# XPixelGroup/DiffBIR

Hardware: NVIDIA B200
Metric: MPix/s end-to-end 50-step restore @512px (higher is better)
Workload: dtype f16 operands / f32 accumulate

## Files before the change

diffbir_b200/csrc/common.cuh:

```cuda
#pragma once
#include <cuda.h>
#include <cuda_runtime.h>
#include <cuda_fp16.h>
#include <cuda_bf16.h>
#include <stdint.h>
#include <stdio.h>

#ifdef DBIR_OPERAND_BF16
typedef __nv_bfloat16 op_t;
typedef __nv_bfloat162 op2_t;
#define DBIR_OPERAND_KIND 0
#define DBIR_UMMA_FMT 1u
__device__ __forceinline__ op_t f2op(float x) { return __float2bfloat16_rn(x); }
__device__ __forceinline__ float op2f(op_t x) { return __bfloat162float(x); }
__device__ __forceinline__ uint32_t pack2(float a, float b) {
  __nv_bfloat162 v = __floats2bfloat162_rn(a, b);
  return *reinterpret_cast<uint32_t*>(&v);
}
__device__ __forceinline__ float2 unpack2(uint32_t u) {
  __nv_bfloat162 v = *reinterpret_cast<__nv_bfloat162*>(&u);
  return __bfloat1622float2(v);
}
#else
typedef __half op_t;
// ... 9 lines not shown
__device__ __forceinline__ float2 unpack2(uint32_t u) {
  __half2 v = *reinterpret_cast<__half2*>(&u);
  return __half22float2(v);
}
#endif

void dbir_set_error(const char* fmt, ...);
#define DBIR_CHECK_CUDA(expr)                                                     \
  do {                                                                            \
    cudaError_t _e = (expr);                                                      \
    if (_e != cudaSuccess) {                                                      \
      dbir_set_error("%s:%d: %s -> %s", __FILE__, __LINE__, #expr,                \
                     cudaGetErrorString(_e));                                     \
      return -1;                                                                  \
    }                                                                             \
  } while (0)
#define DBIR_REQUIRE(cond, ...)                                                   \
  do {                                                                            \
    if (!(cond)) {                                                                \
      dbir_set_error(__VA_ARGS__);                                                \
      return -2;                                                                  \
    }                                                                             \
  } while (0)

int dbir_make_tmap(CUtensorMap* out, const void* base, int rank, const uint64_t* dims,
                   const uint64_t* strides_bytes, const uint32_t* box, int elem_bytes,
                   int swizzle128);
extern "C" int dbir_sm_count(void);

#ifdef __CUDACC__
extern "C" int dbir_pdl_enabled(void);
template <typename... KArgs, typename... Args>
inline cudaError_t dbir_launch_cluster(void (*kernel)(KArgs...), dim3 grid, dim3 block, size_t smem,
                                       cudaStream_t st, unsigned cluster_x, Args&&... args) {
  cudaLaunchConfig_t cfg{};
  cfg.gridDim = grid;
  cfg.blockDim = block;
  cfg.dynamicSmemBytes = smem;
  cfg.stream = st;
  cudaLaunchAttribute attr[2];
  int n = 0;
  if (dbir_pdl_enabled()) {
    attr[n].id = cudaLaunchAttributeProgrammaticStreamSerialization;
    attr[n].val.programmaticStreamSerializationAllowed = 1;
    ++n;
  }
  if (cluster_x > 1) {
    attr[n].id = cudaLaunchAttributeClusterDimension;
    attr[n].val.clusterDim.x = cluster_x;
    attr[n].val.clusterDim.y = 1;
    attr[n].val.clusterDim.z = 1;
    ++n;
  }
  cfg.attrs = attr;
  cfg.numAttrs = n;
  return cudaLaunchKernelEx(&cfg, kernel, static_cast<KArgs>(args)...);
}
template <typename... KArgs, typename... Args>
inline cudaError_t dbir_launch(void (*kernel)(KArgs...), dim3 grid, dim3 block, size_t smem,
                               cudaStream_t st, Args&&... args) {
  return dbir_launch_cluster(kernel, grid, block, smem, st, 1u, static_cast<Args&&>(args)...);
}
__device__ __forceinline__ void pdl_wait() { asm volatile("griddepcontrol.wait;" ::: "memory"); }
__device__ __forceinline__ void pdl_trigger() { asm volatile("griddepcontrol.launch_dependents;" ::: "memory"); }

__device__ __forceinline__ uint32_t smem_u32(const void* p) {
  return static_cast<uint32_t>(__cvta_generic_to_shared(p));
}

__device__ __forceinline__ bool elect_one() {
  uint32_t pred;
  asm volatile(
      "{\n.reg .pred p;\nelect.sync _|p, 0xffffffff;\nselp.u32 %0, 1, 0, p;\n}\n" : "=r"(pred));
  return pred != 0;
}

__device__ __forceinline__ void mbar_init(uint64_t* bar, uint32_t count) {
  asm volatile("mbarrier.init.shared::cta.b64 [%0], %1;" ::"r"(smem_u32(bar)), "r"(count)
               : "memory");
}
__device__ __forceinline__ void fence_mbar_init() {
  asm volatile("fence.mbarrier_init.release.cluster;" ::: "memory");
}
__device__ __forceinline__ void mbar_expect_tx(uint64_t* bar, uint32_t bytes) {
  asm volatile("mbarrier.arrive.expect_tx.shared::cta.b64 _, [%0], %1;" ::"r"(smem_u32(bar)),
               "r"(bytes)
               : "memory");
}
__device__ __forceinline__ void mbar_arrive(uint64_t* bar) {
  asm volatile("mbarrier.arrive.shared::cta.b64 _, [%0];" ::"r"(smem_u32(bar)) : "memory");
}
__device__ __forceinline__ bool mbar_try_wait(uint64_t* bar, uint32_t parity) {
  uint32_t ok;
  asm volatile(
// ... 282 lines not shown
```

diffbir_b200/csrc/gemm_tc.cu:

```cuda
#include "common.cuh"
#include "../../include/diffbir_b200.h"
#include <stdlib.h>
#include <array>
#include <map>
#include <mutex>
#include <utility>
#include <vector>

namespace {

constexpr int BM = 128;
constexpr int BK = 64;
constexpr int A_SUB_BYTES = BM * BK * 2;
constexpr int EPI_TILE_BYTES = 32 * 32 * 4;

struct GemmParams {
  int M, N, num_kb;
  int mode;
  int H, W, NI;
  int bw, bh, bni;
  int tiles_x, tiles_y;
  int cblocks;
  int kw, pad;
  int wbw, wbh;
  int out_kind;
  const float* bias;
  const float* rowvec;
  int rows_per_vec;
  int has_residual;
  float alpha;
  int act;
  float act_param;
  int geglu;
  int bias_per_row;
  int group_span;
  int splits, kb_per_split;
  float* ws;
  unsigned int* tickets;
  long long* dbg;
  float* stats;
  int stats_nslots, stats_rows_per_img, stats_slots_x;
  const char* pf_ptr;
  long long pf_bytes;
};

__device__ __forceinline__ float apply_act(float v, int act, float prm) {
  if (act == 1) return gelu_erf_f(v);
  if (act == 2) return v > 0.f ? v : v * prm;
  return silu_f(v);
}

__device__ __forceinline__ void sts_v4(uint32_t addr, uint32_t a, uint32_t b, uint32_t c, uint32_t d) {
  asm volatile("st.shared.v4.b32 [%0], {%1, %2, %3, %4};" ::"r"(addr), "r"(a), "r"(b), "r"(c), "r"(d) : "memory");
}
__device__ __forceinline__ float4 lds_v4(uint32_t addr) {
  float4 v;
  asm volatile("ld.shared.v4.f32 {%0, %1, %2, %3}, [%4];" : "=f"(v.x), "=f"(v.y), "=f"(v.z), "=f"(v.w) : "r"(addr) : "memory");
  return v;
}
__device__ __forceinline__ void tma_store_2d(const CUtensorMap* m, uint32_t src, int c0, int c1) {
  asm volatile("cp.async.bulk.tensor.2d.global.shared::cta.bulk_group [%0, {%2, %3}], [%1];" ::"l"(
                   reinterpret_cast<uint64_t>(m)), "r"(src), "r"(c0), "r"(c1) : "memory");
}
__device__ __forceinline__ void tma_store_4d(const CUtensorMap* m, uint32_t src, int c0, int c1, int c2, int c3) {
  asm volatile("cp.async.bulk.tensor.4d.global.shared::cta.bulk_group [%0, {%2, %3, %4, %5}], [%1];" ::"l"(
                   reinterpret_cast<uint64_t>(m)), "r"(src), "r"(c0), "r"(c1), "r"(c2), "r"(c3) : "memory");
}
__device__ __forceinline__ void bulk_commit() { asm volatile("cp.async.bulk.commit_group;" ::: "memory"); }
template <int N>
__device__ __forceinline__ void bulk_wait_read() {
  asm volatile("cp.async.bulk.wait_group.read %0;" ::"n"(N) : "memory");
}

struct EpiCtx {
  const CUtensorMap* tm_out;
  const CUtensorMap* tm_res;
  uint32_t epi_base;
  uint32_t res_bar;
  int row0;
  int x, y, n;
  long long stats_base;
  int grp_off;
  __device__ __forceinline__ uint32_t out_buf(int b) const { return epi_base + b * EPI_TILE_BYTES; }
  __device__ __forceinline__ uint32_t res_buf(int b) const { return epi_base + (2 + b) * EPI_TILE_BYTES; }
  __device__ __forceinline__ uint32_t bar(int b) const { return res_bar + b * 8; }
};

__device__ __forceinline__ void mbar_wait_s(uint32_t bar, uint32_t parity) {
  uint32_t ok = 0;
  long long t0 = 0;
// ... 123 lines not shown
    }
    if (lane < ncols)
      *reinterpret_cast<float2*>(p.stats + (e.stats_base + gc0 + lane) * 2) = make_float2(sa, sb);
  }
  if (lane == 0) {
    if (p.mode == 0) tma_store_2d(e.tm_out, e.out_buf(b), gc0, e.row0);
    else tma_store_4d(e.tm_out, e.out_buf(b), gc0, e.x, e.y, e.n);
    bulk_commit();
  }
}

template <int BN, int STAGES, int EW, bool PAIR, int KSUB>
__global__ void __launch_bounds__(64 + 32 * EW, EW == 4 ? 2 : 1)
gemm_tc_kernel(const __grid_constant__ CUtensorMap tma_a, const __grid_constant__ CUtensorMap tma_b,
               const __grid_constant__ CUtensorMap tma_out, const __grid_constant__ CUtensorMap tma_res,
               const GemmParams p) {
  constexpr int B_ROWS = PAIR ? BN / 2 : BN;
  constexpr int B_SUB_BYTES = B_ROWS * BK * 2;
  constexpr int A_STAGE_BYTES = KSUB * A_SUB_BYTES;
  constexpr int B_STAGE_BYTES = KSUB * B_SUB_BYTES;
  constexpr uint32_t TMEM_COLS = BN <= 32 ? 32 : BN <= 64 ? 64 : BN <= 128 ? 128 : 256;
  static_assert(STAGES * (A_STAGE_BYTES + B_STAGE_BYTES) >= EW * 4 * EPI_TILE_BYTES, "epilogue staging must fit in the pipeline stages");
  constexpr int CSTEP = 32 * (EW / 4);
  extern __shared__ uint8_t smem_raw[];
  uint8_t* smem = reinterpret_cast<uint8_t*>((reinterpret_cast<uintptr_t>(smem_raw) + 1023) &
                                             ~static_cast<uintptr_t>(1023));
  uint8_t* sA = smem;
  uint8_t* sB = smem + STAGES * A_STAGE_BYTES;
  uint64_t* full = reinterpret_cast<uint64_t*>(sB + STAGES * B_STAGE_BYTES);
  uint64_t* empty = full + STAGES;
  uint64_t* tmem_full = empty + STAGES;
  uint64_t* res_bars = tmem_full + 1;
  uint32_t* tmem_slot = reinterpret_cast<uint32_t*>(res_bars + 2 * EW);
  uint32_t* split_flag = tmem_slot + 1;

  const int warp = threadIdx.x >> 5;
  const int lane = threadIdx.x & 31;
  const uint32_t cta_rank = PAIR ? cluster_ctarank() : 0u;
  const int m_tile = blockIdx.x;
  const int n_tile = blockIdx.y;
  const int tile_lin = blockIdx.y * gridDim.x + blockIdx.x;
  const int kb0 = blockIdx.z * p.kb_per_split;
  const int kb1 = min(p.num_kb, kb0 + p.kb_per_split);
  long long t_start = 0, t_setup = 0, t_acc = 0;
  if (p.dbg) t_start = clock64();

  int n0 = 0, y0 = 0, x0 = 0;
  if (p.mode == 1) {
    int t = m_tile;
    int tx = t % p.tiles_x; t /= p.tiles_x;
    int ty = t % p.tiles_y; t /= p.tiles_y;
    x0 = tx * p.bw; y0 = ty * p.bh; n0 = t * p.bni;
  }

  int grp_off = 0;
  if (p.group_span > 0) grp_off = ((p.mode == 1 ? n0 : m_tile) / p.group_span) * p.N;

  if (warp == 0 && lane == 0) {
    tma_prefetch_desc(&tma_a);
    tma_prefetch_desc(&tma_b);
    tma_prefetch_desc(&tma_out);
    if (p.has_residual) tma_prefetch_desc(&tma_res);
  }
  if (warp == 1 && lane == 0) {
    for (int s = 0; s < STAGES; ++s) { mbar_init(&full[s], 1); mbar_init(&empty[s], 1); }
    mbar_init(tmem_full, 1);
    for (int i = 0; i < 2 * EW; ++i) mbar_init(&res_bars[i], 1);
    fence_mbar_init();
  }
  if (warp == 2) {
    if constexpr (PAIR) tmem_alloc_pair(tmem_slot, TMEM_COLS);
    else tmem_alloc(tmem_slot, TMEM_COLS);
  }
  tc_fence_before();
  if constexpr (PAIR) cluster_sync_all();
  else __syncthreads();
  tc_fence_after();
// ... 145 lines not shown
      const int vsel = any_row ? __shfl_sync(0xffffffffu, vec_idx, __ffs(vm) - 1) : 0;
      const bool uniform = !p.rowvec || !any_row || __all_sync(0xffffffffu, out_row < 0 || vec_idx == vsel);
      if (uniform) {
        have_pre = true;
#pragma unroll
        for (int i = 0; i < MAX_PRE; ++i) {
          const int col = n_tile * BN + c_first + i * CSTEP + lane;
          float x = 0.f;
          if (c_first + i * CSTEP < BN && col < p.N) {
            if (p.bias) x = __ldg(p.bias + grp_off + col);
            if (p.rowvec && any_row) x += __ldg(p.rowvec + static_cast<long long>(vsel) * p.N + col);
          }
          pre[i] = x;
        }
      }
    }
    constexpr int MAX_G = (BN / 2) / CSTEP + 1;
    float pa[MAX_G], pg[MAX_G];
    if (p.geglu) {
#pragma unroll
      for (int i = 0; i < MAX_G; ++i) {
        const int c = c_first + i * CSTEP + lane;
        const bool live = p.bias && c_first + i * CSTEP < BN / 2 && n_tile * (BN / 2) + c < p.N / 2;
        pa[i] = live ? __ldg(p.bias + grp_off + n_tile * BN + c) : 0.f;
        pg[i] = live ? __ldg(p.bias + grp_off + n_tile * BN + BN / 2 + c) : 0.f;
      }
    }
    mbar_wait(tmem_full, 0);
    tc_fence_after();
    if (p.dbg) t_acc = clock64();
    const uint32_t taddr = tmem_base + (static_cast<uint32_t>(q * 32) << 16);
    e.epi_base = smem_u32(sA) + ew * (4 * EPI_TILE_BYTES);

    constexpr int OUT_COLS = BN;
    const bool finalize = p.splits == 1;
    if (!p.geglu) {
      const int col_base = n_tile * BN;
      if (finalize && p.has_residual) {
#pragma unroll
        for (int c = 0; c < 2; ++c) {
          const int cc = c_first + c * CSTEP;
          if (cc < OUT_COLS && col_base + cc < p.N) epi_issue_residual(p, e, lane, c, col_base + cc);
        }
      }
      int ci = 0;
#pragma unroll 1
      for (int c0 = c_first; c0 < BN; c0 += CSTEP) {
        uint32_t acc[32];
        __syncwarp();
        tmem_ld32(taddr + c0, acc);
        tmem_ld_wait();
        const int gc0 = col_base + c0;
        if (p.splits > 1) {
          float* wcol = p.ws + ((static_cast<long long>(tile_lin) * p.splits + blockIdx.z) * BN + c0) * BM + r;
#pragma unroll
          for (int j = 0; j < 32; ++j) __stcg(wcol + j * BM, __uint_as_float(acc[j]));
          continue;
        }
        if (gc0 >= p.N) continue;
        const int ncols = min(32, p.N - gc0);
        const int ngc = gc0 + 2 * CSTEP;
        float v[32];
#pragma unroll
        for (int j = 0; j < 32; ++j) v[j] = __uint_as_float(acc[j]);
        finish_chunk(p, e, v, lane, ci, gc0, ncols, (c0 + 2 * CSTEP < BN && ngc < p.N) ? ngc : -1, out_row, vec_idx, true,
                     have_pre, pre[(c0 - c_first) / CSTEP]);
        ++ci;
      }
      if (p.splits > 1) {
        __threadfence();
        asm volatile("bar.sync 1, %0;" ::"n"(32 * EW) : "memory");
        if (threadIdx.x == 64) {
          const unsigned int t = atomicAdd(&p.tickets[tile_lin], 1u);
          const bool last = (t == static_cast<unsigned int>(p.splits) - 1);
          if (last) p.tickets[tile_lin] = 0;
          *split_flag = last ? 1u : 0u;
        }
        asm volatile("bar.sync 1, %0;" ::"n"(32 * EW) : "memory");
        if (*split_flag) {
          __threadfence();
          if (p.has_residual) {
#pragma unroll
            for (int c = 0; c < 2; ++c) {
              const int cc = c_first + c * CSTEP;
              if (cc < BN && col_base + cc < p.N) epi_issue_residual(p, e, lane, c, col_base + cc);
            }
          }
          int cj = 0;
#pragma unroll 1
          for (int c0 = c_first; c0 < BN; c0 += CSTEP) {
            const int gc0 = col_base + c0;
            if (gc0 >= p.N) continue;
            const int ncols = min(32, p.N - gc0);
            const int ngc = gc0 + 2 * CSTEP;
            float v[32];
#pragma unroll
            for (int j = 0; j < 32; ++j) v[j] = 0.f;
            for (int z = 0; z < p.splits; ++z) {
              const float* wcol = p.ws + ((static_cast<long long>(tile_lin) * p.splits + z) * BN + c0) * BM + r;
#pragma unroll
              for (int j = 0; j < 32; ++j) v[j] += __ldcg(wcol + j * BM);
            }
            finish_chunk(p, e, v, lane, cj, gc0, ncols, (c0 + 2 * CSTEP < BN && ngc < p.N) ? ngc : -1, out_row, vec_idx, true,
                         have_pre, pre[(c0 - c_first) / CSTEP]);
            ++cj;
          }
        }
      }
    } else {
      constexpr int HB = BN / 2;
      const int n_half = p.N / 2;
      if constexpr (HB % 32 == 0) {
        const uint32_t bb = e.res_buf(0);
#pragma unroll
        for (int i = 0; i < MAX_G; ++i) {
          asm volatile("st.shared.f32 [%0], %1;" ::"r"(bb + (i * 64 + lane) * 4), "f"(pa[i]) : "memory");
          asm volatile("st.shared.f32 [%0], %1;" ::"r"(bb + (i * 64 + 32 + lane) * 4), "f"(pg[i]) : "memory");
        }
        __syncwarp();
        int ci = 0;
#pragma unroll
        for (int i = 0; i < MAX_G; ++i) {
          const int c0 = c_first + i * CSTEP;
          if (c0 >= HB) break;
          uint32_t av[32], ag[32];
          __syncwarp();
          tmem_ld32(taddr + c0, av);
          tmem_ld32(taddr + HB + c0, ag);
          tmem_ld_wait();
          const int gc0 = n_tile * HB + c0;
          if (gc0 >= n_half) continue;
          const int ncols = min(32, n_half - gc0);
          float v[32];
#pragma unroll
          for (int jj = 0; jj < 8; ++jj) {
            const float4 ba = lds_v4(bb + i * 256 + jj * 16), bg = lds_v4(bb + i * 256 + 128 + jj * 16);
            float a0, a1, a2, a3, g0, g1, g2, g3, y0, y1, y2, y3;
            fadd2(a0, a1, __uint_as_float(av[4 * jj]), __uint_as_float(av[4 * jj + 1]), ba.x, ba.y);
            fadd2(a2, a3, __uint_as_float(av[4 * jj + 2]), __uint_as_float(av[4 * jj + 3]), ba.z, ba.w);
            fadd2(g0, g1, __uint_as_float(ag[4 * jj]), __uint_as_float(ag[4 * jj + 1]), bg.x, bg.y);
            fadd2(g2, g3, __uint_as_float(ag[4 * jj + 2]), __uint_as_float(ag[4 * jj + 3]), bg.z, bg.w);
            gelu_erf_f2(g0, g1, y0, y1);
            gelu_erf_f2(g2, g3, y2, y3);
            fmul2(v[4 * jj], v[4 * jj + 1], a0, a1, y0, y1);
            fmul2(v[4 * jj + 2], v[4 * jj + 3], a2, a3, y2, y3);
          }
          finish_chunk(p, e, v, lane, ci, gc0, ncols, -1, out_row, vec_idx, false);
          ++ci;
        }
      }
    }
    if (lane == 0) bulk_wait_read<0>();
    __syncwarp();
    tc_fence_before();
    if (p.dbg && threadIdx.x == 64) {
      long long* d = p.dbg + 8LL * ((static_cast<long long>(blockIdx.z) * gridDim.y + blockIdx.y) * gridDim.x + blockIdx.x);
      d[0] = t_start; d[1] = t_setup; d[2] = t_acc; d[3] = clock64();
    }
  }
  if constexpr (PAIR) cluster_sync_all();
  else __syncthreads();
  if (warp == 2) {
    tc_fence_after();
    if constexpr (PAIR) tmem_dealloc_pair(tmem_base, TMEM_COLS);
    else tmem_dealloc(tmem_base, TMEM_COLS);
  }
}

template <int BN, int STAGES, int EW, bool PAIR = false, int KSUB = 1>
int launch(const CUtensorMap& ta, const CUtensorMap& tb, const CUtensorMap& to, const CUtensorMap& tr,
           const GemmParams& p, dim3 grid, cudaStream_t st) {
  constexpr int smem = STAGES * KSUB * (A_SUB_BYTES + (PAIR ? BN / 2 : BN) * BK * 2) + 1024 + 512;
  static_assert(smem <= 227 * 1024, "pipeline does not fit in shared memory");
  static bool configured = false;
  if (!configured) {
    DBIR_CHECK_CUDA(cudaFuncSetAttribute(gemm_tc_kernel<BN, STAGES, EW, PAIR, KSUB>,
                                         cudaFuncAttributeMaxDynamicSharedMemorySize, smem));
    configured = true;
  }
  DBIR_CHECK_CUDA(dbir_launch_cluster(gemm_tc_kernel<BN, STAGES, EW, PAIR, KSUB>, grid, dim3(64 + 32 * EW), smem, st,
                                      PAIR ? 2u : 1u, ta, tb, to, tr, p));
  return 0;
}

struct TilePlan { int bn, splits, kb_per_split, pair; };

__host__ int plan_ksub(int bn, int pair, bool wide) {
  if (pair) return (bn == 256 && !wide) ? 1 : 2;
  if (bn == 256) return 1;
  return (wide || bn <= 64) ? 2 : 1;
}

struct PlanQuery {
  int m_tiles, N, num_kb, geglu, forced_bn, split_req, pair_req;
  long long ws_floats_avail;
};

template <typename F>
void for_each_plan(const PlanQuery& q, F f) {
  const int cands[5] = {256, 160, 128, 64, 32};
  const int sms = dbir_sm_count();
  static const int pair_env = [] { const char* e = getenv("DBIR_GEMM_PAIR"); return e ? atoi(e) : -1; }();
  const int pair_mode = q.pair_req == 1 ? 1 : q.pair_req == 2 ? 0 : pair_env;
  const bool can_pair = pair_mode != 0 && !(q.m_tiles & 1);
  static const int ragged_wide = [] { const char* e = getenv("DBIR_GEMM_RAGGED_WIDE"); return e ? atoi(e) : 0; }();
  for (int i = 0; i < 10; ++i) {
    const int bn = cands[i % 5];
    const int pair = 1 - i / 5;
    if (pair && (!can_pair || bn < 64)) continue;
    if (!pair && pair_mode == 1 && can_pair && bn >= 64) continue;
    if (q.forced_bn > 0 && bn != q.forced_bn) continue;
    if (q.forced_bn <= 0) {
      if (q.geglu && bn < 64) continue;
      if (bn > 64 && q.N % bn != 0 && !(ragged_wide && q.N > bn)) continue;
    }
    const long long tiles = static_cast<long long>(q.m_tiles) * ((q.N + bn - 1) / bn);
    for (int s = 1; s <= 16; ++s) {
      if (s > 1) {
        if (q.split_req == 1 || q.geglu || q.ws_floats_avail <= 0) break;
        if (q.num_kb / s < 6) break;
        if (tiles > 16384 || tiles * s * 128LL * bn > q.ws_floats_avail) break;
        if (tiles * (s - 1) >= 2LL * sms) break;
      }
      if (q.split_req > 1 && s != q.split_req) continue;
      const int kbs = (q.num_kb + s - 1) / s;
      if (static_cast<long long>(kbs) * (s - 1) >= q.num_kb) continue;
      const long long ctas = tiles * s;
      const bool wide = ctas <= sms;
      const bool two = !wide && (bn <= 160 || pair);
      const int ksub = plan_ksub(bn, pair, wide);
      double ovh = ksub == 2 ? 290.0 : 520.0;
      if (pair) ovh *= 0.92;
      const double mma = 2.0 * bn;
      const long long slots = static_cast<long long>(sms) * (two ? 2 : 1);
      const double waves = static_cast<double>((ctas + slots - 1) / slots);
      double conc = 1.0;
      if (two) conc = ctas >= 2LL * sms ? 2.0 : static_cast<double>(ctas) / sms;
      const double iters = static_cast<double>((kbs + ksub - 1) / ksub) * ksub;
      const double main = iters * (ovh > conc * mma ? ovh : conc * mma);
      double epi = two ? 500.0 + 55.0 * bn : 1500.0 + 28.0 * bn;
      if (s > 1) epi += 30.0 * bn + 6.0 * bn * s;
      if (two) epi *= 0.5;
      f(TilePlan{bn, s, kbs, pair}, waves * (2500.0 + (pair ? 900.0 : 0.0) + main + epi));
    }
  }
}

TilePlan pick_plan(const PlanQuery& q) {
  TilePlan best{64, 1, q.num_kb, 0};
  double best_cost = -1.0;
  for_each_plan(q, [&](const TilePlan& t, double cost) {
    if (best_cost < 0 || cost < best_cost) { best_cost = cost; best = t; }
  });
  return best;
}

using PlanKey = std::array<long long, 20>;
std::mutex g_plan_mu;
std::mutex g_tune_mu;
std::map<PlanKey, TilePlan> g_plan_cache;
int g_tuned_problems = 0;

bool autotune_enabled() {
  static const int on = [] { const char* e = getenv("DBIR_GEMM_AUTOTUNE"); return e ? atoi(e) : 1; }();
  return on != 0;
}

PlanKey make_key(const dbir_gemm_args* a) {
  PlanKey k{};
  int i = 0;
  k[i++] = a->M; k[i++] = a->N; k[i++] = a->K; k[i++] = a->a_mode;
  k[i++] = a->img_n; k[i++] = a->img_h; k[i++] = a->img_w; k[i++] = a->img_c; k[i++] = a->ksize;
  k[i++] = a->out_kind; k[i++] = a->geglu; k[i++] = a->force_bn; k[i++] = a->split_k; k[i++] = a->cta_pair;
  k[i++] = a->residual != nullptr; k[i++] = a->gn_partials != nullptr;
  k[i++] = a->splitk_ws ? a->splitk_ws_bytes : 0;
  k[i++] = a->lda; k[i++] = a->ldo; k[i++] = a->act * 8 + (a->groups > 1 ? a->groups : 1);
  return k;
}

int gemm_impl(const dbir_gemm_args* a, cudaStream_t st, const TilePlan* forced);

struct TuneScratch {
  void* out = nullptr; size_t out_cap = 0;
  void* part = nullptr; size_t part_cap = 0;
  void* flush = nullptr;
  static constexpr size_t FLUSH_BYTES = 192u << 20;
  cudaEvent_t ev[3][2] = {};
  bool ready = false;
};
TuneScratch g_ts;

bool tune_reserve(void** ptr, size_t* cap, size_t need) {
  if (need <= *cap) return true;
  if (*ptr) cudaFree(*ptr);
  *ptr = nullptr; *cap = 0;
  if (cudaMalloc(ptr, need) != cudaSuccess) { cudaGetLastError(); return false; }
  *cap = need;
  return true;
}

bool tune_plan(const dbir_gemm_args* a, cudaStream_t st, const PlanQuery& q, TilePlan* out_plan) {
  TuneScratch& ts = g_ts;
  if (!ts.ready) {
    if (cudaMalloc(&ts.flush, TuneScratch::FLUSH_BYTES) != cudaSuccess) { cudaGetLastError(); return false; }
    for (auto& e : ts.ev) for (auto& x : e) if (cudaEventCreate(&x) != cudaSuccess) return false;
    ts.ready = true;
  }
  const int eb = a->out_kind == 0 ? 4 : 2;
// ... 41 lines not shown
  if (!autotune_enabled()) return pick_plan(q);
  const PlanKey key = make_key(a);
  {
    std::lock_guard<std::mutex> lk(g_plan_mu);
    auto it = g_plan_cache.find(key);
    if (it != g_plan_cache.end()) return it->second;
  }
  TilePlan plan = pick_plan(q);
  cudaStreamCaptureStatus cs = cudaStreamCaptureStatusNone;
  if (cudaStreamIsCapturing(st, &cs) != cudaSuccess) { cudaGetLastError(); return plan; }
  if (cs != cudaStreamCaptureStatusNone) return plan;
  std::lock_guard<std::mutex> tune_lk(g_tune_mu);
  {
    std::lock_guard<std::mutex> lk(g_plan_mu);
    auto it = g_plan_cache.find(key);
    if (it != g_plan_cache.end()) return it->second;
  }
  TilePlan tuned = plan;
  if (tune_plan(a, st, q, &tuned)) plan = tuned;
  std::lock_guard<std::mutex> lk(g_plan_mu);
  g_plan_cache[key] = plan;
  ++g_tuned_problems;
  return plan;
}

}

extern "C" int dbir_gemm(const dbir_gemm_args* a, void* stream) {
  return gemm_impl(a, reinterpret_cast<cudaStream_t>(stream), nullptr);
}
extern "C" int dbir_gemm_model_plan(int32_t m_tiles, int32_t N, int32_t num_kb, int32_t geglu, int32_t force_bn,
                                    int32_t split_k, int32_t cta_pair, int64_t ws_floats, int32_t* out) {
  DBIR_REQUIRE(m_tiles > 0 && N > 0 && num_kb > 0 && out, "dbir_gemm_model_plan: bad arguments");
  const TilePlan t = pick_plan(PlanQuery{m_tiles, N, num_kb, geglu, force_bn, split_k, cta_pair, ws_floats});
  out[0] = t.bn; out[1] = t.splits; out[2] = t.kb_per_split; out[3] = t.pair;
  return 0;
}
extern "C" int32_t dbir_gemm_tuned_problems(void) { return g_tuned_problems; }
extern "C" void dbir_gemm_clear_plans(void) {
  std::lock_guard<std::mutex> lk(g_plan_mu);
  g_plan_cache.clear();
}

namespace {
int gemm_impl(const dbir_gemm_args* a, cudaStream_t st, const TilePlan* forced) {
  DBIR_REQUIRE(a != nullptr, "dbir_gemm: null args");
  DBIR_REQUIRE(a->M > 0 && a->N > 0 && a->K > 0, "dbir_gemm: bad shape M=%d N=%d K=%d", a->M,
               a->N, a->K);
  DBIR_REQUIRE(a->a && a->b && a->out, "dbir_gemm: null pointer");
  DBIR_REQUIRE(a->K % 8 == 0, "dbir_gemm: K=%d must be a multiple of 8 (16-byte rows)", a->K);
  DBIR_REQUIRE(!a->out2, "dbir_gemm: out2 is not supported by the TMA-store epilogue");
  const int eb = a->out_kind == 0 ? 4 : 2;
  DBIR_REQUIRE((a->ldo * eb) % 16 == 0, "dbir_gemm: output row stride must be a multiple of 16 bytes (ldo=%lld)",
               (long long)a->ldo);
  DBIR_REQUIRE(!a->residual || a->ldr % 4 == 0, "dbir_gemm: residual row stride must be a multiple of 4");

  GemmParams p{};
  p.M = a->M; p.N = a->N;
  p.mode = a->a_mode;
  p.out_kind = a->out_kind;
  p.bias = a->bias; p.rowvec = a->rowvec;
  p.rows_per_vec = a->rows_per_vec > 0 ? a->rows_per_vec : a->M;
  p.has_residual = a->residual != nullptr;
  p.alpha = a->alpha; p.act = a->act; p.act_param = a->act_param; p.geglu = a->geglu;
  p.bias_per_row = a->bias_per_row;
  const int groups = a->groups > 1 ? a->groups : 1;
  if (groups > 1) {
// ... 69 lines not shown
    }
    const int wbw = bw < 32 ? bw : 32;
    const int wbh = bh < 32 / wbw ? bh : 32 / wbw;
    const int wbn = 32 / (wbw * wbh);
    p.wbw = wbw; p.wbh = wbh;
    uint64_t odims[4] = {static_cast<uint64_t>(n_out), static_cast<uint64_t>(W), static_cast<uint64_t>(H),
                         static_cast<uint64_t>(NI)};
    uint64_t ostr[3] = {static_cast<uint64_t>(a->ldo) * eb, static_cast<uint64_t>(W) * a->ldo * eb,
                        static_cast<uint64_t>(H) * W * a->ldo * eb};
    uint32_t obox[4] = {32, static_cast<uint32_t>(wbw), static_cast<uint32_t>(wbh), static_cast<uint32_t>(wbn)};
    if (dbir_make_tmap(&to, a->out, 4, odims, ostr, obox, eb, eb == 4 ? 1 : 2)) return -3;
    tr = to;
    if (a->residual) {
      uint64_t rstr[3] = {static_cast<uint64_t>(a->ldr) * 4, static_cast<uint64_t>(W) * a->ldr * 4,
                          static_cast<uint64_t>(H) * W * a->ldr * 4};
      if (dbir_make_tmap(&tr, a->residual, 4, odims, rstr, obox, 4, 1)) return -3;
    }
  }

  if (a->gn_partials) {
    DBIR_REQUIRE(a->out_kind == 0 && !a->geglu, "dbir_gemm: gn_partials needs an fp32, non-GEGLU output");
    p.stats = reinterpret_cast<float*>(a->gn_partials);
    if (a->a_mode == 0) {
      DBIR_REQUIRE(a->gn_rows_per_img > 0 && a->gn_rows_per_img % 32 == 0 && a->M % a->gn_rows_per_img == 0,
                   "dbir_gemm: gn_partials in matrix mode needs rows-per-image that is a multiple of 32");
      p.stats_rows_per_img = a->gn_rows_per_img;
      p.stats_nslots = a->gn_rows_per_img / 32;
    } else {
      DBIR_REQUIRE(p.bw * p.bh >= 32, "dbir_gemm: gn_partials needs images of at least 32 pixels");
      p.stats_slots_x = (p.W + p.wbw - 1) / p.wbw;
      p.stats_nslots = p.stats_slots_x * ((p.H + p.wbh - 1) / p.wbh);
    }
  }
  constexpr long long TICKET_FLOATS = 16384;
  const long long ws_floats = a->splitk_ws ? a->splitk_ws_bytes / 4 - TICKET_FLOATS : 0;
  int pair_req = a->cta_pair;
  if (groups > 1 && ((m_tiles / groups) & 1)) pair_req = 2;
  const PlanQuery pq{m_tiles, a->N, p.num_kb, a->geglu, a->force_bn, a->split_k, pair_req, ws_floats};
  const TilePlan plan = forced ? *forced : choose_plan(a, st, pq);
  const int bn = plan.bn;
  p.splits = plan.splits;
  p.kb_per_split = plan.kb_per_split;
  if (plan.splits > 1) {
    p.tickets = reinterpret_cast<unsigned int*>(a->splitk_ws);
    p.ws = reinterpret_cast<float*>(a->splitk_ws) + TICKET_FLOATS;
  }
  {
    const long long ldb = a->ldb > 0 ? a->ldb : a->K;
    uint64_t dims[2] = {static_cast<uint64_t>(a->K), static_cast<uint64_t>(a->N) * groups};
    uint64_t strides[1] = {static_cast<uint64_t>(ldb) * 2};
    uint32_t box[2] = {BK, static_cast<uint32_t>(plan.pair ? bn / 2 : bn)};
    if (dbir_make_tmap(&tb, a->b, 2, dims, strides, box, 2, 1)) return -3;
  }
  dim3 grid(m_tiles, (a->N + bn - 1) / bn, plan.splits);
  static const int wide_mode = [] { const char* e = getenv("DBIR_GEMM_WIDE"); return e ? atoi(e) : -1; }();
  const bool wide = wide_mode >= 0 ? wide_mode != 0
                                   : static_cast<long long>(grid.x) * grid.y * grid.z <= dbir_sm_count();
#define DBIR_GO(BN_, ST_, EW_, PAIR_, KS_) return launch<BN_, ST_, EW_, PAIR_, KS_>(ta, tb, to, tr, p, grid, st)
  if (plan.pair) {
    switch (bn) {
      case 64:  if (wide) DBIR_GO(64, 4, 8, true, 2);  else DBIR_GO(64, 2, 4, true, 2);
      case 128: if (wide) DBIR_GO(128, 4, 8, true, 2); else DBIR_GO(128, 2, 4, true, 2);
      case 160: if (wide) DBIR_GO(160, 4, 8, true, 2); else DBIR_GO(160, 2, 4, true, 2);
      case 256: if (wide) DBIR_GO(256, 3, 8, true, 2); else DBIR_GO(256, 3, 4, true, 1);
      default:
        dbir_set_error("dbir_gemm: unsupported paired tile width %d", bn);
        return -2;
    }
  }
  switch (bn) {
    case 32:  if (wide) DBIR_GO(32, 4, 8, false, 2);  else DBIR_GO(32, 2, 4, false, 2);
    case 64:  if (wide) DBIR_GO(64, 4, 8, false, 2);  else DBIR_GO(64, 2, 4, false, 2);
    case 128: if (wide) DBIR_GO(128, 3, 8, false, 2); else DBIR_GO(128, 3, 4, false, 1);
    case 160: if (wide) DBIR_GO(160, 3, 8, false, 2); else DBIR_GO(160, 3, 4, false, 1);
    case 256: DBIR_GO(256, 4, 8, false, 1);
    default:
      dbir_set_error("dbir_gemm: unsupported tile width %d", bn);
      return -2;
  }
// ... 17 lines not shown
```

diffbir_b200/engine/cldm.py:

```python
from __future__ import annotations

import os
from typing import Dict, List, Optional, Sequence

import torch

from .. import arch, lib
from .common import Workspace, f32, geglu_tile, op16, pack_conv3x3, pack_geglu, pack_linear

HEAD_DIM = 64


class _Net:

    def __init__(self, sd: Dict[str, torch.Tensor], cfg: dict, controlnet: bool, device):
        self.cfg = cfg
        self.plan = arch.unet_plan(cfg, controlnet)
        self.controlnet = controlnet
        self.dev = device
        self.w: Dict[str, torch.Tensor] = {}
        shapes = arch.unet_shapes(cfg, controlnet)
        missing = [k for k in shapes if k not in sd]
        if missing:
            raise KeyError(f"checkpoint is missing {len(missing)} keys, e.g. {missing[:3]}")
# ... 162 lines not shown
                offs["c" + l.prefix] = total
                total += nb * l.cout
        table = torch.empty(S, total, dtype=torch.float32, device=self.dev)
        emb_dim = 4 * self.mc
        for net, tag in ((self.unet, "u"), (self.cnet, "c")):
            te = torch.empty(S, self.mc, dtype=torch.float32, device=self.dev)
            lib.timestep_embedding(t, S, self.mc, te)
            h1 = torch.empty(S, emb_dim, dtype=torch.float32, device=self.dev)
            lib.linear_f32(te, self.mc, S, self.mc, net.w["time_embed.0.weight"],
                           net.w["time_embed.0.bias"], emb_dim, h1, emb_dim, silu_out=True)
            emb_act = torch.empty(S, emb_dim, dtype=torch.float32, device=self.dev)
            lib.linear_f32(h1, emb_dim, S, emb_dim, net.w["time_embed.2.weight"],
                           net.w["time_embed.2.bias"], emb_dim, emb_act, emb_dim, silu_out=True)
            tmp = torch.empty(S, max(l.cout for l in net.res_layers), dtype=torch.float32, device=self.dev)
            for l in net.res_layers:
                o = offs[tag + l.prefix]
                y = tmp[:, : l.cout]
                lib.linear_f32(emb_act, emb_dim, S, emb_dim, net.w[l.prefix + "emb.w"],
                               net.w[l.prefix + "emb.b"], l.cout, y, tmp.shape[1])
                table[:, o:o + nb * l.cout] = y.repeat(1, nb)
        self.emb_table = table
        self.emb_offsets = offs
        self.emb_nb = nb
        if self.emb_cur is None or self.emb_cur.numel() != total:
            self.emb_cur = torch.empty(total, dtype=torch.float32, device=self.dev)
            self._graphs.clear()
        self.timesteps = list(timesteps)
        self._ts_key = key

    def load_step(self, step_idx: int):
        self.emb_cur.copy_(self.emb_table[step_idx])

    def _gemm(self, tag: str, a, b, *args, **kw):
        ws = self.ws.get(tag + ":splitk", (16 * 1024 * 1024 + 16384,), torch.float32, zero=True)
        seq = self._wseq.setdefault(tag, [])
        i = self._wpos.get(tag, 0)
        wbytes = b.numel() * b.element_size()
        if i < len(seq):
            if seq[i][0] != b.data_ptr():
                del seq[i:]
        if i >= len(seq):
            seq.append((b.data_ptr(), wbytes))
        self._wpos[tag] = i + 1
        pf = None
        if self.prefetch_weights and i + 1 < len(seq):
            pf = seq[i + 1]
        if self.batch_invariant:
            kw.setdefault("split_k", 1)
        lib.gemm(a, b, *args, splitk_ws=ws, prefetch=pf, **kw)

    def _emb(self, tag: str, l: arch.Layer, nb: int) -> torch.Tensor:
        if tag == "g":
            o = self.emb_offsets["u" + l.prefix]
            assert self.emb_offsets["c" + l.prefix] == o + (nb // 2) * l.cout
            return self.emb_cur[o:o + nb * l.cout]
        o = self.emb_offsets[tag + l.prefix]
        return self.emb_cur[o:o + nb * l.cout]

    def _gn(self, tag, src1, src2, c1, c2, nb, h, w, eps, gamma, beta, out16, silu, out_raw=None, G=1):
        ws = self.ws
        stats = ws.get(tag + ":gn_stats", (nb * 64,), torch.float32)
        p1 = self._part.get(src1.data_ptr())
        p2 = self._part.get(src2.data_ptr()) if src2 is not None else None
        if self.fuse_gn_stats and p1 is not None and (src2 is None or p2 is not None):
            lib.gn_finalize(p1[0], p1[1], c1, p2[0] if p2 else None, p2[1] if p2 else 0, c2, nb, h * w, eps, stats)
        else:
            wsp = ws.get(tag + ":gn_ws", (lib.gn_workspace_floats(nb, h * w, c1 + c2),), torch.float32, zero=True)
# ... 260 lines not shown
```

Before: 0.9006.

## Reduce split-K partials through cluster DSMEM instead of global workspace tickets

Replaces the global-memory split-K reduction, which wrote partials to a workspace and used an atomic ticket to pick a last CTA, with a cluster-based reduction. The split CTAs are launched as a cluster along z, stage their partials in shared memory, and each CTA sums its own slice of column chunks via distributed shared memory before finishing it. This removes the global round trip and serialised last-CTA epilogue, but adds cluster launch constraints, caps splits at 8, and forbids split-K with CTA pairs and geglu. The planner cost model is updated to match.

```diff
diff --git a/diffbir_b200/csrc/common.cuh b/diffbir_b200/csrc/common.cuh
--- a/diffbir_b200/csrc/common.cuh
+++ b/diffbir_b200/csrc/common.cuh
@@ -65,7 +65,7 @@
 extern "C" int dbir_pdl_enabled(void);
 template <typename... KArgs, typename... Args>
 inline cudaError_t dbir_launch_cluster(void (*kernel)(KArgs...), dim3 grid, dim3 block, size_t smem,
-                                       cudaStream_t st, unsigned cluster_x, Args&&... args) {
+                                       cudaStream_t st, dim3 cluster, Args&&... args) {
   cudaLaunchConfig_t cfg{};
   cfg.gridDim = grid;
   cfg.blockDim = block;
@@ -78,11 +78,11 @@
     attr[n].val.programmaticStreamSerializationAllowed = 1;
     ++n;
   }
-  if (cluster_x > 1) {
+  if (cluster.x * cluster.y * cluster.z > 1) {
     attr[n].id = cudaLaunchAttributeClusterDimension;
-    attr[n].val.clusterDim.x = cluster_x;
-    attr[n].val.clusterDim.y = 1;
-    attr[n].val.clusterDim.z = 1;
+    attr[n].val.clusterDim.x = cluster.x;
+    attr[n].val.clusterDim.y = cluster.y;
+    attr[n].val.clusterDim.z = cluster.z;
     ++n;
   }
   cfg.attrs = attr;
@@ -92,7 +92,7 @@
 template <typename... KArgs, typename... Args>
 inline cudaError_t dbir_launch(void (*kernel)(KArgs...), dim3 grid, dim3 block, size_t smem,
                                cudaStream_t st, Args&&... args) {
-  return dbir_launch_cluster(kernel, grid, block, smem, st, 1u, static_cast<Args&&>(args)...);
+  return dbir_launch_cluster(kernel, grid, block, smem, st, dim3(1), static_cast<Args&&>(args)...);
 }
 __device__ __forceinline__ void pdl_wait() { asm volatile("griddepcontrol.wait;" ::: "memory"); }
 __device__ __forceinline__ void pdl_trigger() { asm volatile("griddepcontrol.launch_dependents;" ::: "memory"); }
diff --git a/diffbir_b200/csrc/gemm_tc.cu b/diffbir_b200/csrc/gemm_tc.cu
--- a/diffbir_b200/csrc/gemm_tc.cu
+++ b/diffbir_b200/csrc/gemm_tc.cu
@@ -13,6 +13,7 @@
 constexpr int BK = 64;
 constexpr int A_SUB_BYTES = BM * BK * 2;
 constexpr int EPI_TILE_BYTES = 32 * 32 * 4;
+constexpr int MAX_SPLITS = 8;
 
 struct GemmParams {
   int M, N, num_kb;
@@ -35,8 +36,6 @@
   int bias_per_row;
   int group_span;
   int splits, kb_per_split;
-  float* ws;
-  unsigned int* tickets;
   long long* dbg;
   float* stats;
   int stats_nslots, stats_rows_per_img, stats_slots_x;
@@ -56,6 +55,11 @@
 __device__ __forceinline__ float4 lds_v4(uint32_t addr) {
   float4 v;
   asm volatile("ld.shared.v4.f32 {%0, %1, %2, %3}, [%4];" : "=f"(v.x), "=f"(v.y), "=f"(v.z), "=f"(v.w) : "r"(addr) : "memory");
+  return v;
+}
+__device__ __forceinline__ float4 ld_dsmem_v4(uint32_t cluster_addr) {
+  float4 v;
+  asm volatile("ld.shared::cluster.v4.f32 {%0, %1, %2, %3}, [%4];" : "=f"(v.x), "=f"(v.y), "=f"(v.z), "=f"(v.w) : "r"(cluster_addr) : "memory");
   return v;
 }
 __device__ __forceinline__ void tma_store_2d(const CUtensorMap* m, uint32_t src, int c0, int c1) {
@@ -245,17 +249,15 @@
   uint64_t* tmem_full = empty + STAGES;
   uint64_t* res_bars = tmem_full + 1;
   uint32_t* tmem_slot = reinterpret_cast<uint32_t*>(res_bars + 2 * EW);
-  uint32_t* split_flag = tmem_slot + 1;
 
   const int warp = threadIdx.x >> 5;
   const int lane = threadIdx.x & 31;
   const uint32_t cta_rank = PAIR ? cluster_ctarank() : 0u;
   const int m_tile = blockIdx.x;
   const int n_tile = blockIdx.y;
-  const int tile_lin = blockIdx.y * gridDim.x + blockIdx.x;
   const int kb0 = blockIdx.z * p.kb_per_split;
   const int kb1 = min(p.num_kb, kb0 + p.kb_per_split);
-  long long t_start = 0, t_setup = 0, t_acc = 0;
+  long long t_start = 0, t_setup = 0, t_acc = 0, t_red = 0;
   if (p.dbg) t_start = clock64();
 
   int n0 = 0, y0 = 0, x0 = 0;
@@ -467,15 +469,13 @@
     const uint32_t taddr = tmem_base + (static_cast<uint32_t>(q * 32) << 16);
     e.epi_base = smem_u32(sA) + ew * (4 * EPI_TILE_BYTES);
 
-    constexpr int OUT_COLS = BN;
-    const bool finalize = p.splits == 1;
-    if (!p.geglu) {
+    if (!p.geglu && p.splits == 1) {
       const int col_base = n_tile * BN;
-      if (finalize && p.has_residual) {
+      if (p.has_residual) {
 #pragma unroll
         for (int c = 0; c < 2; ++c) {
           const int cc = c_first + c * CSTEP;
-          if (cc < OUT_COLS && col_base + cc < p.N) epi_issue_residual(p, e, lane, c, col_base + cc);
+          if (cc < BN && col_base + cc < p.N) epi_issue_residual(p, e, lane, c, col_base + cc);
         }
       }
       int ci = 0;
@@ -486,12 +486,6 @@
         tmem_ld32(taddr + c0, acc);
         tmem_ld_wait();
         const int gc0 = col_base + c0;
-        if (p.splits > 1) {
-          float* wcol = p.ws + ((static_cast<long long>(tile_lin) * p.splits + blockIdx.z) * BN + c0) * BM + r;
-#pragma unroll
-          for (int j = 0; j < 32; ++j) __stcg(wcol + j * BM, __uint_as_float(acc[j]));
-          continue;
-        }
         if (gc0 >= p.N) continue;
         const int ncols = min(32, p.N - gc0);
         const int ngc = gc0 + 2 * CSTEP;
@@ -502,45 +496,76 @@
                      have_pre, pre[(c0 - c_first) / CSTEP]);
         ++ci;
       }
-      if (p.splits > 1) {
-        __threadfence();
-        asm volatile("bar.sync 1, %0;" ::"n"(32 * EW) : "memory");
-        if (threadIdx.x == 64) {
-          const unsigned int t = atomicAdd(&p.tickets[tile_lin], 1u);
-          const bool last = (t == static_cast<unsigned int>(p.splits) - 1);
-          if (last) p.tickets[tile_lin] = 0;
-          *split_flag = last ? 1u : 0u;
-        }
-        asm volatile("bar.sync 1, %0;" ::"n"(32 * EW) : "memory");
-        if (*split_flag) {
-          __threadfence();
-          if (p.has_residual) {
-#pragma unroll
-            for (int c = 0; c < 2; ++c) {
-              const int cc = c_first + c * CSTEP;
-              if (cc < BN && col_base + cc < p.N) epi_issue_residual(p, e, lane, c, col_base + cc);
-            }
-          }
-          int cj = 0;
+    } else if (!PAIR && !p.geglu) {
+      constexpr int NCH = BN / 32;
+      constexpr uint32_t CH_BYTES = 128 * 32 * 4;
+      const int S = p.splits, z = blockIdx.z;
+      const int lo = z * NCH / S, hi = (z + 1) * NCH / S;
+      const uint32_t part = smem_u32(sA) + STAGES * (A_STAGE_BYTES + B_STAGE_BYTES) - NCH * CH_BYTES;
+      const int sw = lane & 7;
+      const uint32_t rrow = static_cast<uint32_t>(r) * 128;
+      auto pos_of = [&](int j, int zz) { return static_cast<uint32_t>((j + NCH - (zz + 1) * NCH / S) % NCH); };
 #pragma unroll 1
-          for (int c0 = c_first; c0 < BN; c0 += CSTEP) {
-            const int gc0 = col_base + c0;
-            if (gc0 >= p.N) continue;
-            const int ncols = min(32, p.N - gc0);
-            const int ngc = gc0 + 2 * CSTEP;
-            float v[32];
-#pragma unroll
-            for (int j = 0; j < 32; ++j) v[j] = 0.f;
-            for (int z = 0; z < p.splits; ++z) {
-              const float* wcol = p.ws + ((static_cast<long long>(tile_lin) * p.splits + z) * BN + c0) * BM + r;
-#pragma unroll
-              for (int j = 0; j < 32; ++j) v[j] += __ldcg(wcol + j * BM);
-            }
-            finish_chunk(p, e, v, lane, cj, gc0, ncols, (c0 + 2 * CSTEP < BN && ngc < p.N) ? ngc : -1, out_row, vec_idx, true,
-                         have_pre, pre[(c0 - c_first) / CSTEP]);
-            ++cj;
+      for (int c0 = c_first; c0 < BN; c0 += CSTEP) {
+        uint32_t acc[32];
+        __syncwarp();
+        tmem_ld32(taddr + c0, acc);
+        tmem_ld_wait();
+        const uint32_t dst = part + pos_of(c0 / 32, z) * CH_BYTES + rrow;
+#pragma unroll
+        for (int j = 0; j < 8; ++j) sts_v4(dst + ((j ^ sw) << 4), acc[4 * j], acc[4 * j + 1], acc[4 * j + 2], acc[4 * j + 3]);
+      }
+      __syncwarp();
+      cluster_sync_all();
+#pragma unroll 1
+      for (int j = lo + (ew >> 2); j < hi; j += EW / 4) {
+        float v[32];
+#pragma unroll
+        for (int k = 0; k < 32; ++k) v[k] = 0.f;
+#pragma unroll 1
+        for (int zz = 0; zz < S; ++zz) {
+          const uint32_t src = mapa_u32(part + pos_of(j, zz) * CH_BYTES + rrow, static_cast<uint32_t>(zz));
+#pragma unroll
+          for (int k = 0; k < 8; ++k) {
+            const float4 t = ld_dsmem_v4(src + ((k ^ sw) << 4));
+            v[4 * k] += t.x; v[4 * k + 1] += t.y; v[4 * k + 2] += t.z; v[4 * k + 3] += t.w;
           }
         }
+        const uint32_t dst = part + pos_of(j, z) * CH_BYTES + rrow;
+#pragma unroll
+        for (int k = 0; k < 8; ++k)
+          sts_v4(dst + ((k ^ sw) << 4), __float_as_uint(v[4 * k]), __float_as_uint(v[4 * k + 1]),
+                 __float_as_uint(v[4 * k + 2]), __float_as_uint(v[4 * k + 3]));
+      }
+      __syncwarp();
+      cluster_sync_all();
+      if (p.dbg) t_red = clock64();
+      const int col_base = n_tile * BN;
+      const int first = lo + (ew >> 2);
+      if (p.has_residual) {
+#pragma unroll
+        for (int c = 0; c < 2; ++c) {
+          const int jj = first + c * (EW / 4);
+          if (jj < hi && col_base + jj * 32 < p.N) epi_issue_residual(p, e, lane, c, col_base + jj * 32);
+        }
+      }
+      int ci = 0;
+#pragma unroll 1
+      for (int j = first; j < hi; j += EW / 4) {
+        const int gc0 = col_base + j * 32;
+        if (gc0 >= p.N) continue;
+        const int ncols = min(32, p.N - gc0);
+        const int jn = j + 2 * (EW / 4);
+        const uint32_t src = part + pos_of(j, z) * CH_BYTES + rrow;
+        float v[32];
+#pragma unroll
+        for (int k = 0; k < 8; ++k) {
+          const float4 t = lds_v4(src + ((k ^ sw) << 4));
+          v[4 * k] = t.x; v[4 * k + 1] = t.y; v[4 * k + 2] = t.z; v[4 * k + 3] = t.w;
+        }
+        finish_chunk(p, e, v, lane, ci, gc0, ncols, (jn < hi && col_base + jn * 32 < p.N) ? col_base + jn * 32 : -1,
+                     out_row, vec_idx, true);
+        ++ci;
       }
     } else {
       constexpr int HB = BN / 2;
@@ -590,8 +615,13 @@
     tc_fence_before();
     if (p.dbg && threadIdx.x == 64) {
       long long* d = p.dbg + 8LL * ((static_cast<long long>(blockIdx.z) * gridDim.y + blockIdx.y) * gridDim.x + blockIdx.x);
-      d[0] = t_start; d[1] = t_setup; d[2] = t_acc; d[3] = clock64();
-    }
+      d[0] = t_start; d[1] = t_setup; d[2] = t_acc; d[3] = clock64(); d[4] = t_red;
+    }
+  }
+  if (!PAIR && p.splits > 1 && warp < 2) {
+    __syncwarp();
+    cluster_sync_all();
+    cluster_sync_all();
   }
   if constexpr (PAIR) cluster_sync_all();
   else __syncthreads();
@@ -605,8 +635,16 @@
 template <int BN, int STAGES, int EW, bool PAIR = false, int KSUB = 1>
 int launch(const CUtensorMap& ta, const CUtensorMap& tb, const CUtensorMap& to, const CUtensorMap& tr,
            const GemmParams& p, dim3 grid, cudaStream_t st) {
-  constexpr int smem = STAGES * KSUB * (A_SUB_BYTES + (PAIR ? BN / 2 : BN) * BK * 2) + 1024 + 512;
+  constexpr int stage_bytes = STAGES * KSUB * (A_SUB_BYTES + (PAIR ? BN / 2 : BN) * BK * 2);
+  constexpr int smem = stage_bytes + 1024 + 512;
   static_assert(smem <= 227 * 1024, "pipeline does not fit in shared memory");
+  if (p.splits > 1) {
+    const int nch = BN / 32, own = (nch + p.splits - 1) / p.splits;
+    if (PAIR || p.geglu || p.splits > MAX_SPLITS || nch * 16384 > stage_bytes || (EW * 4 + own * 16) * 1024 > stage_bytes) {
+      dbir_set_error("dbir_gemm: no split-K over %d splits for tile <%d, %d, %d, %d>", p.splits, BN, STAGES, EW, int(PAIR));
+      return -2;
+    }
+  }
   static bool configured = false;
   if (!configured) {
     DBIR_CHECK_CUDA(cudaFuncSetAttribute(gemm_tc_kernel<BN, STAGES, EW, PAIR, KSUB>,
@@ -614,7 +652,7 @@
     configured = true;
   }
   DBIR_CHECK_CUDA(dbir_launch_cluster(gemm_tc_kernel<BN, STAGES, EW, PAIR, KSUB>, grid, dim3(64 + 32 * EW), smem, st,
-                                      PAIR ? 2u : 1u, ta, tb, to, tr, p));
+                                      dim3(PAIR ? 2u : 1u, 1u, static_cast<unsigned>(p.splits)), ta, tb, to, tr, p));
   return 0;
 }
 
@@ -628,7 +666,7 @@
 
 struct PlanQuery {
   int m_tiles, N, num_kb, geglu, forced_bn, split_req, pair_req;
-  long long ws_floats_avail;
+  bool allow_split;
 };
 
 template <typename F>
@@ -643,19 +681,19 @@
     const int bn = cands[i % 5];
     const int pair = 1 - i / 5;
     if (pair && (!can_pair || bn < 64)) continue;
-    if (!pair && pair_mode == 1 && can_pair && bn >= 64) continue;
+    if (!pair && pair_mode == 1 && can_pair && bn >= 64 && q.split_req <= 1) continue;
     if (q.forced_bn > 0 && bn != q.forced_bn) continue;
     if (q.forced_bn <= 0) {
       if (q.geglu && bn < 64) continue;
       if (bn > 64 && q.N % bn != 0 && !(ragged_wide && q.N > bn)) continue;
     }
     const long long tiles = static_cast<long long>(q.m_tiles) * ((q.N + bn - 1) / bn);
-    for (int s = 1; s <= 16; ++s) {
+    for (int s = 1; s <= MAX_SPLITS; ++s) {
       if (s > 1) {
-        if (q.split_req == 1 || q.geglu || q.ws_floats_avail <= 0) break;
+        if (q.split_req == 1 || q.geglu || !q.allow_split || pair) break;
         if (q.num_kb / s < 6) break;
-        if (tiles > 16384 || tiles * s * 128LL * bn > q.ws_floats_avail) break;
         if (tiles * (s - 1) >= 2LL * sms) break;
+        if (bn == 160 && s == 2 && tiles * s > sms) continue;
       }
       if (q.split_req > 1 && s != q.split_req) continue;
       const int kbs = (q.num_kb + s - 1) / s;
@@ -674,7 +712,10 @@
       const double iters = static_cast<double>((kbs + ksub - 1) / ksub) * ksub;
       const double main = iters * (ovh > conc * mma ? ovh : conc * mma);
       double epi = two ? 500.0 + 55.0 * bn : 1500.0 + 28.0 * bn;
-      if (s > 1) epi += 30.0 * bn + 6.0 * bn * s;
+      if (s > 1) {
+        const int own = (bn / 32 + s - 1) / s;
+        epi = (two ? 500.0 + 55.0 * 32 * own : 1500.0 + 28.0 * 32 * own) + 8.0 * bn + 1000.0 + 150.0 * s * own;
+      }
       if (two) epi *= 0.5;
       f(TilePlan{bn, s, kbs, pair}, waves * (2500.0 + (pair ? 900.0 : 0.0) + main + epi));
     }
@@ -708,7 +749,7 @@
   k[i++] = a->img_n; k[i++] = a->img_h; k[i++] = a->img_w; k[i++] = a->img_c; k[i++] = a->ksize;
   k[i++] = a->out_kind; k[i++] = a->geglu; k[i++] = a->force_bn; k[i++] = a->split_k; k[i++] = a->cta_pair;
   k[i++] = a->residual != nullptr; k[i++] = a->gn_partials != nullptr;
-  k[i++] = a->splitk_ws ? a->splitk_ws_bytes : 0;
+  k[i++] = a->splitk_ws != nullptr;
   k[i++] = a->lda; k[i++] = a->ldo; k[i++] = a->act * 8 + (a->groups > 1 ? a->groups : 1);
   return k;
 }
@@ -816,7 +857,7 @@
 extern "C" int dbir_gemm_model_plan(int32_t m_tiles, int32_t N, int32_t num_kb, int32_t geglu, int32_t force_bn,
                                     int32_t split_k, int32_t cta_pair, int64_t ws_floats, int32_t* out) {
   DBIR_REQUIRE(m_tiles > 0 && N > 0 && num_kb > 0 && out, "dbir_gemm_model_plan: bad arguments");
-  const TilePlan t = pick_plan(PlanQuery{m_tiles, N, num_kb, geglu, force_bn, split_k, cta_pair, ws_floats});
+  const TilePlan t = pick_plan(PlanQuery{m_tiles, N, num_kb, geglu, force_bn, split_k, cta_pair, ws_floats > 0});
   out[0] = t.bn; out[1] = t.splits; out[2] = t.kb_per_split; out[3] = t.pair;
   return 0;
 }
@@ -952,19 +993,14 @@
       p.stats_nslots = p.stats_slots_x * ((p.H + p.wbh - 1) / p.wbh);
     }
   }
-  constexpr long long TICKET_FLOATS = 16384;
-  const long long ws_floats = a->splitk_ws ? a->splitk_ws_bytes / 4 - TICKET_FLOATS : 0;
+
   int pair_req = a->cta_pair;
   if (groups > 1 && ((m_tiles / groups) & 1)) pair_req = 2;
-  const PlanQuery pq{m_tiles, a->N, p.num_kb, a->geglu, a->force_bn, a->split_k, pair_req, ws_floats};
+  const PlanQuery pq{m_tiles, a->N, p.num_kb, a->geglu, a->force_bn, a->split_k, pair_req, a->splitk_ws != nullptr};
   const TilePlan plan = forced ? *forced : choose_plan(a, st, pq);
   const int bn = plan.bn;
   p.splits = plan.splits;
   p.kb_per_split = plan.kb_per_split;
-  if (plan.splits > 1) {
-    p.tickets = reinterpret_cast<unsigned int*>(a->splitk_ws);
-    p.ws = reinterpret_cast<float*>(a->splitk_ws) + TICKET_FLOATS;
-  }
   {
     const long long ldb = a->ldb > 0 ? a->ldb : a->K;
     uint64_t dims[2] = {static_cast<uint64_t>(a->K), static_cast<uint64_t>(a->N) * groups};
diff --git a/diffbir_b200/engine/cldm.py b/diffbir_b200/engine/cldm.py
--- a/diffbir_b200/engine/cldm.py
+++ b/diffbir_b200/engine/cldm.py
@@ -218,7 +218,7 @@
         self.emb_cur.copy_(self.emb_table[step_idx])
 
     def _gemm(self, tag: str, a, b, *args, **kw):
-        ws = self.ws.get(tag + ":splitk", (16 * 1024 * 1024 + 16384,), torch.float32, zero=True)
+        ws = self.ws.get(tag + ":splitk", (4,), torch.float32)
         seq = self._wseq.setdefault(tag, [])
         i = self._wpos.get(tag, 0)
         wbytes = b.numel() * b.element_size()
```

Result: no change. 0.8930 (median of 6 runs) (-0.8%).
